# gaoyubin/EasyDarwin

Measured on AMD Instinct MI355X. Metric: relayed RTP packets/sec (whole node) + achieved HBM GB/s, 1080p H.264 fan-out, higher is better.
Workload: dtype u8

## Files before the change

### easydarwin_amd/csrc/edgpu_device.h

```cpp
#pragma once
#include <stdint.h>

namespace edgpu {

enum : uint32_t {
    kMaxPacket = 2060,
    kSlotWordsMax = 129,
    kIngestThreads = 256,
    kMaxTracks = 16,
    kMaxSendersPerSession = 2 * kMaxTracks,
};

enum : uint32_t {
    kSndRtcpPort = 1u << 0,
    kSndRtcpKind = 1u << 1,
    kSndVideo    = 1u << 2,
    kSndH264     = 1u << 3,
    kSndAudio    = 1u << 4,
};

struct PktMeta {
    uint64_t vbyte;
    uint64_t id;
    int64_t  arrival;
// ... 233 lines not shown

struct TickTotals {
    unsigned long long relayed_packets;
    unsigned long long relayed_bytes;
    unsigned long long arena_bytes;
    unsigned long long ing_pk[2], ing_b[2];
    int status;
    unsigned int nwork;
    unsigned long long cum_relayed_packets;
    unsigned long long cum_relayed_bytes;
    unsigned long long cum_fanout_in_bytes;
    unsigned long long cum_ingested_packets;
    unsigned long long cum_ingested_bytes;
    int ingest_status;
    unsigned int fan_next;
    unsigned int _pad;
    unsigned long long pass_bytes[2];
    unsigned int pass_desc[2];
    unsigned int pass_next[2];
    unsigned int pass_slot;
    unsigned int stream_errors;
    unsigned long long cum_lost_passes;
    unsigned int grow_count;
    unsigned int _pad_g;
};

struct GrowReq {
    uint32_t sender;
    uint32_t pk_log2;
    uint32_t bytes_log2;
    uint32_t _pad;
    uint64_t tail, head;
};
constexpr uint32_t kMaxGrow = 1024;
constexpr uint32_t kNoPass = 0xFFFFFFFFu;

struct TickParams {
    int64_t  now;
    int64_t  over_buffer_ms;
    uint64_t arena_bytes;
    uint32_t max_desc;
    uint32_t nsenders;
    uint32_t nsubs;
    uint32_t nsub_blocks;
    uint32_t chunk;
    uint32_t pass_ord;
    uint32_t pass_id;
    uint32_t grow_on;
    uint32_t grow_max_pk;
    uint64_t grow_max_bytes;
    uint32_t* grow_flag;
};

}
```

### easydarwin_amd/csrc/edgpu_engine.cpp

```cpp
#include <hip/hip_runtime.h>

#include <algorithm>
#include <cctype>
#include <chrono>
#include <thread>
#include <cstdio>
#include <cstdlib>
#include <cstring>
#include <map>
#include <mutex>
#include <string>
#include <vector>

#include <sched.h>

#include "edgpu.h"
#include "edgpu_device.h"

#include "edgpu_params.h"

namespace edgpu {
hipError_t launch_ingest(const IngestParams& p, uint32_t nseg, hipStream_t st);
hipError_t launch_blocked(const BlockedParams& p, hipStream_t st);
hipError_t launch_first_packet_info(const FirstInfoQuery* q, FirstInfoResult* r, const SenderDev* senders,
// ... 250 lines not shown
    uint64_t work_cap_needed = 0;
    void* d_null = nullptr;

    DevVec<SessionDev> d_sessions;
    DevVec<SenderDev> d_senders;
    DevVec<StreamDev> d_streams;
    DevVec<StatDev> d_stats;
    uint32_t n_stats = 0;
    struct TapHost { void* rec = nullptr; void* unit = nullptr; uint64_t cap = 0; uint32_t sender = 0; };
    DevVec<TapDev> d_taps;
    std::map<uint32_t, TapHost> taps;
    std::vector<std::pair<uint32_t, uint64_t>> tap_grown;
    bool tap_list_dirty = false;
    DevVec<uint32_t> d_tap_list, d_tap_items;
    DevVec<uint8_t> d_tap_out;
    DevVec<edgpu_tap_unit> d_tap_units;
    DevVec<edgpu_tap_stream> d_tap_streams;
    TapPlace* d_tap_place = nullptr;
    DevVec<uint8_t> d_ts_es, d_ts_out;
    DevVec<edgpu_tap_unit> d_ts_units_in;
    DevVec<TsRange> d_ts_ranges;
    DevVec<edgpu_ts_state> d_ts_states;
    DevVec<TsRec> d_ts_recs;
    DevVec<uint32_t> d_ts_base;
    DevVec<edgpu_ts_unit> d_ts_rows;
    uint8_t* d_ts_fixed = nullptr;
    DevVec<SubDev> d_subs;
    DevVec<uint32_t> d_sub_index;
    DevVec<uint32_t> d_sub_range;
    DevVec<uint32_t> d_sub_pos;
    DevVec<FanSub> d_fansub;
    DevVec<edgpu_substream_out> d_sub_out;
    DevVec<FanWork> d_work;
    DevVec<uint64_t> d_blk_bytes;
    DevVec<uint32_t> d_blk_count;
    DevVec<uint64_t> d_blk_maxb;
    DevVec<uint32_t> d_blk_maxc;
    bool index_dirty = true;
    uint32_t pass_ord = 0, pass_id = 0;
    int passes_more = 0;
    int tick_variant = 0;
    uint64_t fanout_passes = 0;

    edgpu_pkt_desc* d_desc = nullptr;
    uint32_t* d_seg = nullptr;
    uint32_t* d_seg_sess = nullptr;
    uint8_t* d_blob = nullptr;
    struct PinStage {
        edgpu_pkt_desc* desc = nullptr;
        uint32_t* seg = nullptr;
        uint32_t* sess = nullptr;
        uint8_t* blob = nullptr;
        hipEvent_t copied = nullptr;
        hipEvent_t consumed = nullptr;
        bool issued = false;
        uint64_t prestaged = 0;
    } pin[2];
    hipStream_t h2d = nullptr;
    int pin_next = 0;
    std::mutex pin_mu;
    int pend_stage = -1;
    const uint32_t* pend_seg = nullptr;
    const uint32_t* pend_seg_sess = nullptr;
    uint32_t pend_nseg = 0;
    bool pending = false;

    uint8_t* d_arena = nullptr;
    edgpu_out_desc* d_out_desc = nullptr;
    std::vector<uint32_t> carry_len;
    DevVec<uint8_t> d_carry;
// ... 189 lines not shown
    if (dmalloc(&x->d_seg, sizeof(uint32_t) * ((size_t)c.max_batch_packets + 1)) != hipSuccess) return bad("seg staging");
    if (dmalloc(&x->d_seg_sess, sizeof(uint32_t) * (size_t)c.max_batch_packets) != hipSuccess) return bad("seg staging");
    if (dmalloc(&x->d_arena, c.out_arena_bytes) != hipSuccess) return bad("fan-out arena");
    if (dmalloc(&x->d_out_desc, sizeof(edgpu_out_desc) * (size_t)c.max_out_packets) != hipSuccess) return bad("descriptors");
    if (dmalloc(&x->d_totals, sizeof(TickTotals)) != hipSuccess) return bad("totals");
    if (dmalloc(&x->d_grow, sizeof(GrowReq) * kMaxGrow) != hipSuccess) return bad("ring growth requests");
    if (hipHostMalloc((void**)&x->h_grow_flag, 64, hipHostMallocMapped) != hipSuccess ||
        hipHostGetDevicePointer((void**)&x->d_grow_flag, x->h_grow_flag, 0) != hipSuccess)
        return bad("ring growth flag");
    *x->h_grow_flag = 0;
    if (hipMalloc(&x->d_null, 4096) != hipSuccess || hipMemset(x->d_null, 0, 4096) != hipSuccess) return bad("null ring");
    {
        TickTotals t0;
        memset(&t0, 0, sizeof(t0));
        t0.pass_next[0] = t0.pass_next[1] = kNoPass;
        if (hipMemcpy(x->d_totals, &t0, sizeof(t0), hipMemcpyHostToDevice) != hipSuccess) return bad("totals");
    }
    if (const char* v = getenv("EDGPU_FANOUT")) x->fanout_variant = atoi(v);
    if (const char* v = getenv("EDGPU_TCP_WALK"))
        x->tcp_walk = !strcmp(v, "serial") || !strcmp(v, "1") ? 1u : !strcmp(v, "seg") || !strcmp(v, "2") ? 2u : 0u;
    if (const char* v = getenv("EDGPU_TCP_SEG")) x->tcp_seg = (uint32_t)std::max(atoi(v), 1);
    *out = x;
    return EDGPU_OK;
}

int edgpu_ctx_destroy(edgpu_ctx* x) {
    if (!x) return EDGPU_OK;
    (void)hipSetDevice(x->device);
    if (x->stream) (void)hipStreamSynchronize(x->stream);
    x->rings.release();
    if (x->d_null) (void)hipFree(x->d_null);
    x->d_sessions.release(); x->d_senders.release(); x->d_streams.release(); x->d_stats.release(); x->d_subs.release();
    x->d_sub_index.release(); x->d_sub_range.release(); x->d_sub_pos.release(); x->d_fansub.release(); x->d_sub_out.release(); x->d_work.release();
    x->d_blk_bytes.release(); x->d_blk_count.release(); x->d_blk_maxb.release(); x->d_blk_maxc.release();
    x->d_img_plan.release();
    for (auto& t : x->taps) { (void)hipFree(t.second.rec); (void)hipFree(t.second.unit); }
    x->d_taps.release(); x->d_tap_list.release(); x->d_tap_items.release(); x->d_tap_out.release();
    x->d_tap_units.release(); x->d_tap_streams.release();
    if (x->d_tap_place) (void)hipFree(x->d_tap_place);
    x->d_ts_es.release(); x->d_ts_out.release(); x->d_ts_units_in.release(); x->d_ts_ranges.release();
    x->d_ts_states.release(); x->d_ts_recs.release(); x->d_ts_base.release(); x->d_ts_rows.release();
    if (x->d_ts_fixed) (void)hipFree(x->d_ts_fixed);
    x->d_carry.release(); x->d_tcp_groups.release(); x->d_tcp_reads.release(); x->d_tcp_chunk_group.release();
    x->d_tcp_ncand.release(); x->d_tcp_cands.release(); x->d_tcp_links.release(); x->d_tcp_chunkres.release();
    x->d_tcp_results.release(); x->d_tcp_offs.release(); x->d_tcp_stage.release(); x->d_blocked.release();
    x->d_gather_reg.release(); x->d_gather_off.release(); x->d_arrivals.release(); x->d_sources.release(); x->d_row_sel.release(); x->d_rows.release();
    x->d_act_blk.release(); x->d_act_q.release(); x->d_act_rows.release();
    if (x->d_fpi_q) (void)hipFree(x->d_fpi_q);
    if (x->d_fpi_r) (void)hipFree(x->d_fpi_r);
    if (x->h_fpi_q) (void)hipHostFree(x->h_fpi_q);
    if (x->h_fpi_r) (void)hipHostFree(x->h_fpi_r);
    if (x->h_stage) (void)hipHostFree(x->h_stage);
    if (x->h_grow_flag) (void)hipHostFree(x->h_grow_flag);
    if (x->d_tcp_src) (void)hipFree(x->d_tcp_src);
    if (x->d_tcp_tot) (void)hipFree(x->d_tcp_tot);
    if (x->d_tcp_raw) (void)hipFree(x->d_tcp_raw);
    if (x->d_img_status) (void)hipFree(x->d_img_status);
    for (void* p : {(void*)x->d_desc, (void*)x->d_seg, (void*)x->d_seg_sess,
                    (void*)x->d_blob, (void*)x->d_arena, (void*)x->d_out_desc, (void*)x->d_totals, (void*)x->d_grow})
        if (p) (void)hipFree(p);
    for (auto& w : x->hist) for (auto& s : w) for (auto& e : s) if (e) (void)hipEventDestroy(e);
    if (x->h2d) (void)hipStreamSynchronize(x->h2d);
    for (auto& st : x->pin) {
        for (void* p : {(void*)st.desc, (void*)st.seg, (void*)st.sess, (void*)st.blob}) if (p) (void)hipFree(p);
        if (st.copied) (void)hipEventDestroy(st.copied);
        if (st.consumed) (void)hipEventDestroy(st.consumed);
    }
// ... 836 lines not shown
    }
    return true;
}

static int rebuild_index(edgpu_ctx* x) {
    const uint32_t nsub = (uint32_t)x->sub_sender.size();
    std::vector<uint32_t> range(2 * (size_t)x->nsenders, 0);
    for (uint32_t i = 0; i < nsub; i++)
        if (x->sub_active[i]) range[2 * (size_t)x->sub_sender[i] + 1]++;
    uint32_t total = 0;
    for (uint32_t s = 0; s < x->nsenders; s++) {
        const uint32_t c = range[2 * (size_t)s + 1];
        range[2 * (size_t)s] = total;
        range[2 * (size_t)s + 1] = total;
        total += c;
    }
    std::vector<uint32_t> idx(total);
    std::vector<uint32_t> pos(nsub, 0xFFFFFFFFu);
    for (uint32_t i = 0; i < nsub; i++)
        if (x->sub_active[i]) {
            const uint32_t k = range[2 * (size_t)x->sub_sender[i] + 1]++;
            idx[k] = i;
            pos[i] = k;
        }
    HIP_CHECK(x->d_sub_index.reserve(std::max<size_t>(idx.size(), 1), x->stream));
    HIP_CHECK(x->d_fansub.reserve(std::max<size_t>(idx.size(), 1), x->stream));
    HIP_CHECK(x->d_sub_pos.reserve(std::max<size_t>(nsub, 1), x->stream));
    if (nsub) HIP_CHECK(hipMemcpyAsync(x->d_sub_pos.ptr, pos.data(), nsub * 4, hipMemcpyHostToDevice, x->stream));
    HIP_CHECK(x->d_sub_range.reserve(std::max<size_t>(range.size(), 2), x->stream));
    if (!idx.empty()) HIP_CHECK(hipMemcpyAsync(x->d_sub_index.ptr, idx.data(), idx.size() * 4, hipMemcpyHostToDevice, x->stream));
    if (!range.empty()) HIP_CHECK(hipMemcpyAsync(x->d_sub_range.ptr, range.data(), range.size() * 4, hipMemcpyHostToDevice, x->stream));
    const uint32_t nblk = (nsub + 255) / 256;
    HIP_CHECK(x->d_sub_out.reserve(std::max<uint32_t>(nsub, 1), x->stream));
    HIP_CHECK(x->d_blk_bytes.reserve(std::max<uint32_t>(nblk, 1), x->stream));
    HIP_CHECK(x->d_blk_count.reserve(std::max<uint32_t>(nblk, 1), x->stream));
    HIP_CHECK(x->d_blk_maxb.reserve(std::max<uint32_t>(nblk, 1), x->stream));
    HIP_CHECK(x->d_blk_maxc.reserve(std::max<uint32_t>(nblk, 1), x->stream));
    HIP_CHECK(x->d_work.reserve(std::max<uint64_t>(x->work_cap_needed, 1), x->stream));
    HIP_CHECK(wsync(x, x->stream));
    x->index_dirty = false;
    return EDGPU_OK;
}

static int enqueue_ingest(edgpu_ctx* x, const edgpu_pkt_desc* dd, uint32_t n, const uint32_t* ds, const uint32_t* dss,
                          uint32_t nseg, const uint8_t* db, bool host_src, const TcpParams* tcp = nullptr,
                          bool deframed = false) {
    IngestParams p;
    p.host_epoch = host_src ? ++x->ingest_epoch : 0u;
    if (!host_src) ++x->ingest_epoch;
    x->host_epoch_last = p.host_epoch;
    p.desc = dd; p.seg_off = ds; p.seg_sess = dss; p.blob = db;
    p.src_addr = tcp ? tcp->src_addr : nullptr;
    p.sessions = x->d_sessions.ptr; p.senders = x->d_senders.ptr; p.streams = x->d_streams.ptr;
    p.npk = n; p.spec_min = x->cfg.ingest_spec_min;
    p.totals = x->d_totals;
    x->ing_slot ^= 1u;
    p.ing_slot = x->ing_slot;
    p.recv_time = x->cfg.reflector_use_in_packet_receive_time;
    p.max_future_ms = (int64_t)(uint32_t)(x->cfg.reflector_in_packet_max_receive_sec * 1000u);
    p.tcp_groups = tcp ? tcp->groups : nullptr;
    p.tcp_chunkres = tcp ? tcp->chunkres : nullptr;
    p.tcp_offs = tcp ? tcp->offs : nullptr;
    p.tcp_reads = tcp ? tcp->reads : nullptr;
    p.tcp_raw = tcp ? tcp->raw : nullptr;
    p.tcp_stage = tcp ? tcp->stage : nullptr;
    HIP_CHECK(hist_mark(x, 2, 0));
    if (tcp && !deframed) HIP_CHECK(launch_deframe(*tcp, x->stream));
    HIP_CHECK(launch_ingest(p, nseg, x->stream));
    HIP_CHECK(hist_mark(x, 2, 1));
    if (x->n_stats) {
// ... 294 lines not shown
}

int edgpu_keyframe_index(edgpu_ctx* x) {
    if (!x) return fail(EDGPU_BAD_ARGUMENT, "ctx is NULL");
    if (!x->pending) return fail(EDGPU_ERR, "no ingested batch pending a keyframe index");
    DEVICE_ENTER(x);
    x->kf_share = false;
    if (x->aux) {
        HIP_CHECK(hipEventRecord(x->ev_kf, x->stream));
        x->kf_recorded = true;
    }
    if (x->pend_stage >= 0) {
        HIP_CHECK(hipEventRecord(x->pin[x->pend_stage].consumed, x->stream));
        x->pend_stage = -1;
    }
    x->pending = false;
    return EDGPU_OK;
}

static int pick_fanout_variant(const edgpu_ctx* x) {
    if (x->fanout_variant >= 0) return x->fanout_variant;
    constexpr uint64_t kBurstRows = 4096;
    const bool burst = x->joined_rows >= kBurstRows && x->joined_rows * 4 >= x->sub_sender.size();
    return fanout_default(x->n_rw + x->n_tcp > 0 || burst);
}

static PlanParams plan_params(edgpu_ctx* x, int64_t now_ms) {
    const uint32_t nsub = x->tick_nsubs;
    PlanParams p;
    p.senders = x->d_senders.ptr; p.subs = x->d_subs.ptr; p.sub_index = x->d_sub_index.ptr;
    p.sub_pos = x->d_sub_pos.ptr; p.sub_range = x->d_sub_range.ptr; p.fansub = x->d_fansub.ptr;
    p.sub_out = x->d_sub_out.ptr;
    p.work = x->d_work.ptr;
    p.blk_bytes = x->d_blk_bytes.ptr; p.blk_count = x->d_blk_count.ptr;
    p.blk_maxb = x->d_blk_maxb.ptr; p.blk_maxc = x->d_blk_maxc.ptr;
    p.sessions = x->d_sessions.ptr;
    p.totals = x->d_totals;
    p.T.now = now_ms;
    p.T.over_buffer_ms = (int64_t)x->cfg.reflector_buffer_size_sec * 1000;
    p.T.arena_bytes = x->cfg.out_arena_bytes;
    p.T.max_desc = x->cfg.max_out_packets;
    p.T.nsenders = x->nsenders;
    p.T.nsubs = nsub;
    p.T.nsub_blocks = (nsub + 255) / 256;
    p.T.chunk = (uint32_t)fanout_chunk(x->tick_variant);
    p.T.pass_ord = x->pass_ord;
    p.T.pass_id = x->pass_id;
    p.grow = x->d_grow;
    p.T.grow_on = x->cfg.ring_growth;
    p.T.grow_max_pk = x->cfg.max_ring_packets;
    p.T.grow_max_bytes = x->cfg.max_ring_bytes;
    p.T.grow_flag = x->d_grow_flag;
    return p;
}

static int launch_copy_pass(edgpu_ctx* x, edgpu_fanout_result* out) {
    FanoutParams f;
    f.senders = x->d_senders.ptr; f.sub_range = x->d_sub_range.ptr; f.subs = x->d_subs.ptr;
    f.sub_index = x->d_sub_index.ptr; f.work = x->d_work.ptr; f.fansub = x->d_fansub.ptr;
    f.arena = x->d_arena; f.desc = x->d_out_desc;
    f.arena_words = x->cfg.out_arena_bytes / 16;
    f.max_desc = x->cfg.max_out_packets;
    f.totals = x->d_totals;
    hipStream_t cs = x->stream;
    HIP_CHECK(hist_mark(x, 0, 0, cs));
    HIP_CHECK(launch_fanout(f, x->tick_variant, x->num_cus, cs));
    HIP_CHECK(hist_mark(x, 0, 1, cs));
    x->fanout_passes++;
    x->passes_more = -1;
    if (out) {
        out->arena = f.arena;
        out->desc = f.desc;
        out->substreams = x->d_sub_out.ptr;
        out->n_substreams = x->tick_nsubs;
    }
    return EDGPU_OK;
}

int edgpu_fanout(edgpu_ctx* x, int64_t now_ms, edgpu_fanout_result* out) {
    if (!x) return fail(EDGPU_BAD_ARGUMENT, "ctx is NULL");
    if (x->pending) return fail(EDGPU_ERR, "edgpu_keyframe_index must run after edgpu_ingest");
    if (int r = owed_pass(x, "edgpu_fanout")) return r;
    DEVICE_ENTER(x);
    for (const auto& f : x->free_pending) x->free_subs[f.first].push_back(f.second);
    x->free_pending.clear();
    if (x->index_dirty) { int r = rebuild_index(x); if (r) return r; }
    x->tick_nsubs = (uint32_t)x->sub_sender.size();
    x->last_now = now_ms;
    queue_source_reports(x, now_ms);
    x->tick_variant = pick_fanout_variant(x);
    x->joined_rows = 0;
    x->pass_ord = 0;
    x->pass_id = 0;
    const PlanParams p = plan_params(x, now_ms);
    HIP_CHECK(hist_mark(x, 1, 0));
    HIP_CHECK(launch_plan(p, x->stream));
    if (int r = launch_copy_pass(x, out)) return r;
    if (x->timing >= EDGPU_TIMING_ALL) {
        const uint32_t s1 = x->hist_n[1];
        x->tick_end[s1 % edgpu_ctx::kHist] = x->last_seq[0];
        x->last_seq[1] = s1;
        x->hist_n[1] = s1 + 1;
    }
    x->fanout_launches++;
    x->timed_fanout = true;
    return EDGPU_OK;
}

int edgpu_fanout_next(edgpu_ctx* x, edgpu_fanout_result* out, uint32_t* launched) {
    if (!x || !launched) return fail(EDGPU_BAD_ARGUMENT, "NULL argument");
    *launched = 0;
    if (x->fanout_launches == 0) return fail(EDGPU_ERR, "no fan-out tick");
    DEVICE_ENTER(x);
    TickTotals t;
    if (int r = read_totals(x, &t)) return r;
    note_grow(x, t);
    if (t.status) {
        x->passes_more = 0;
        return fail(t.status, "the tick failed");
    }
    const uint32_t next = t.pass_next[x->pass_ord & 1u];
    if (next == kNoPass) {
        x->passes_more = 0;
        return EDGPU_OK;
    }
    x->pass_ord++;
    x->pass_id = next;
    const PlanParams p = plan_params(x, x->last_now);
    HIP_CHECK(launch_plan_pass(p, x->stream));
// ... 954 lines not shown
```

### easydarwin_amd/csrc/edgpu_kernels.hip

```cpp
#include <hip/hip_runtime.h>
#include <stdint.h>
#include "edgpu.h"
#include "edgpu_device.h"
#include "edgpu_params.h"
#include "edgpu_bytes.h"

namespace edgpu {

typedef unsigned int u32x4 __attribute__((ext_vector_type(4)));

__device__ __forceinline__ u32x4 ing_ld(const u32x4* p) { return *p; }
__device__ __forceinline__ void ing_st(u32x4* p, u32x4 v) { *p = v; }

__device__ __forceinline__ uint32_t be16(const uint8_t* p) { return (uint32_t)p[0] << 8 | p[1]; }
__device__ __forceinline__ uint32_t be32(const uint8_t* p) {
    return (uint32_t)p[0] << 24 | (uint32_t)p[1] << 16 | (uint32_t)p[2] << 8 | p[3];
}

__device__ __forceinline__ uint32_t slot_header(uint32_t len) {
    return 0x24u | ((len >> 8) & 0xFF) << 16 | (len & 0xFF) << 24;
}

__device__ bool key_frame_first_packet(const uint8_t* p, uint32_t len) {
    if (len < 20) return false;
// ... 694 lines not shown
    return lo;
}
__device__ uint64_t wave_first_arrival_at(const SenderDev& D, const PktMeta* meta, uint64_t lo, uint64_t hi, int64_t cut) {
    if (!D.rt_nonmono)
        return wave_lower_bound_meta(meta, D.pk_mask, lo, hi, [&](const PktMeta& m) { return m.arrival >= cut; });
    const uint64_t lane = threadIdx.x & 63;
    for (uint64_t b = lo; b < hi; b += 64) {
        const uint64_t i = b + lane;
        const unsigned long long t = __ballot(i < hi && meta[i & D.pk_mask].arrival >= cut ? 1 : 0);
        if (t) return b + (uint64_t)(__ffsll(t) - 1);
    }
    return hi;
}

__device__ __forceinline__ void reset_tick_totals(TickTotals* t) {
    t->relayed_packets = 0; t->relayed_bytes = 0; t->arena_bytes = 0;
    t->status = 0; t->nwork = 0; t->fan_next = 0; t->stream_errors = 0;
    if (t->pass_next[t->pass_slot & 1u] != kNoPass) t->cum_lost_passes++;
    t->pass_slot = 0;
    for (int k = 0; k < 2; k++) { t->pass_bytes[k] = 0; t->pass_desc[k] = 0; t->pass_next[k] = kNoPass; }
    t->grow_count = 0;
}

__global__ void k_totals_reset(TickTotals* t, int which) {
    if (threadIdx.x != 0) return;
    if (which == 0) reset_tick_totals(t);
    else for (int k = 0; k < 2; k++) { t->ing_pk[k] = 0; t->ing_b[k] = 0; }
}

__device__ __forceinline__ void mark_stream_error(const PlanParams& P, uint32_t session) {
    if (atomicOr(&P.sessions[session].errors, kStreamRingOverflow) == 0u) atomicAdd(&P.totals->stream_errors, 1u);
}

__global__ __launch_bounds__(256) void k_plan_senders(PlanParams P) {
    if (blockIdx.x == 0 && threadIdx.x == 0) reset_tick_totals(P.totals);
    const uint32_t s = blockIdx.x * (blockDim.x / 64) + threadIdx.x / 64;
    if (s >= P.T.nsenders) return;
    SenderDev& D = P.senders[s];
    const PktMeta* meta = reinterpret_cast<const PktMeta*>(D.meta);
    const uint64_t head = D.head;
    const uint64_t pk_cap = (uint64_t)D.pk_mask + 1;
    const uint64_t byte_cap = ((uint64_t)D.word_mask + 1) * 16;
    uint64_t lo = head > pk_cap ? head - pk_cap : 0;
    lo = max(lo, D.floor);
    const uint64_t vend = D.vbyte_end, vhigh = max(vend, D.vclob);
    const uint64_t tail = wave_lower_bound_meta(meta, D.pk_mask, lo, head,
                                                [&](const PktMeta& m) { return vhigh - m.vbyte <= byte_cap; });
    int64_t ns = -1;
    if (D.key >= 0) {
        ns = D.key;
        if ((uint64_t)ns < tail) ns = -2;
    } else if (head > tail) {
        const int64_t cutoff = P.T.now - P.T.over_buffer_ms;
        const uint64_t f = wave_first_arrival_at(D, meta, tail, head, cutoff);
        if (f < head) ns = (f == tail && tail > D.floor) ? -2 : (int64_t)f;
    }
    if (P.T.grow_on && head > tail) {
        const uint64_t held_b = vend - meta[tail & D.pk_mask].vbyte;
        if (2 * (head - tail) > pk_cap || 2 * held_b > byte_cap) {
            const int64_t age_cut = P.T.now - 10 * P.T.over_buffer_ms;
            uint64_t r = wave_first_arrival_at(D, meta, tail, head, age_cut);
            if (D.key >= 0 && (uint64_t)D.key >= tail) r = min(r, (uint64_t)D.key);
            if (D.umin >= tail) r = min(r, D.umin);
            const uint64_t need_pk = head - r;
            const uint64_t need_b = r < head ? vend - meta[r & D.pk_mask].vbyte : 0;
            uint64_t want_pk = pk_cap, want_b = byte_cap;
            while (2 * need_pk > want_pk && want_pk < P.T.grow_max_pk) want_pk *= 2;
            while (2 * need_b > want_b && want_b < P.T.grow_max_bytes) want_b *= 2;
            if ((threadIdx.x & 63) == 0 && (want_pk > pk_cap || want_b > byte_cap)) {
                const uint32_t k = atomicAdd(&P.totals->grow_count, 1u);
                if (k < kMaxGrow)
                    P.grow[k] = GrowReq{s, (uint32_t)(63 - __clzll((long long)want_pk)),
                                        (uint32_t)(63 - __clzll((long long)want_b)), 0u, tail, head};
                if (k == 0 && P.T.grow_flag) *(volatile uint32_t*)P.T.grow_flag = 1u;
            }
        }
    }
    if ((threadIdx.x & 63) == 0) {
        D.tail = tail;
        D.new_start = ns;
        D.umin = head;
    }
}

template <typename T>
__global__ __launch_bounds__(256) void k_ring_move(const T* __restrict__ src, uint64_t smask, T* __restrict__ dst,
                                                   uint64_t dmask, uint64_t lo, uint64_t n) {
    for (uint64_t i = (uint64_t)blockIdx.x * 256 + threadIdx.x; i < n; i += (uint64_t)gridDim.x * 256) {
        const uint64_t v = lo + i;
        dst[v & dmask] = src[v & smask];
    }
}

__global__ __launch_bounds__(256) void k_plan_subs(PlanParams P) {
    const uint32_t q = blockIdx.x * blockDim.x + threadIdx.x;
    uint64_t bytes = 0;
    uint32_t count = 0;
    if (q < P.T.nsubs) {
        SubDev& Q = P.subs[q];
        Q.nonempty = 0; Q.count = 0; Q.bytes = 0;
        Q.was_new = Q.active && Q.bookmark < 0;
        if (Q.active) {
            SenderDev& D = P.senders[Q.sender];
            const PktMeta* meta = reinterpret_cast<const PktMeta*>(D.meta);
            const uint64_t head = D.head;
            bool have = false;
            uint64_t a = 0;
            Q.prev_last_id = Q.last_id;
            Q.prev_has_last = Q.has_last;
            Q.prev_sent_any = Q.sent_any;
            if (Q.bookmark >= 0) {
                a = (uint64_t)Q.bookmark + (Q.resume_at ? 0u : 1u);
                if (Q.rtp_info && Q.kind == 0 && !Q.has_last && (Q.sent_any || P.subs[q + 1].sent_any))
                    a = (uint64_t)Q.bookmark;
                have = true;
                if (a < D.tail && a < head) { mark_stream_error(P, D.session); a = D.tail; }
            } else if (D.new_start >= 0) {
                a = (uint64_t)D.new_start;
                have = true;
                if (Q.has_last)
                    a = lower_bound_meta(meta, D.pk_mask, a, head,
                                         [&](const PktMeta& m) { return m.id > Q.last_id; });
            } else if (D.new_start == -2) {
                mark_stream_error(P, D.session);
            }
            if (have) {
                if (Q.rtp_info && Q.kind == 0 && !Q.sent_any && !P.subs[q + 1].sent_any) {
                    while (a < head) {
                        const PktMeta m = meta[a & D.pk_mask];
                        if (m.len != 0 && m.seq >= Q.first_seq) break;
                        a++;
                    }
                }
                if (a < head) {
                    const PktMeta m = meta[a & D.pk_mask];
                    Q.a = a;
                    Q.vstart = m.vbyte;
                    Q.vcstart = m.vcount;
                    bytes = D.vbyte_end - m.vbyte;
                    count = D.vcount_end - m.vcount;
                    Q.bytes = bytes;
                    Q.count = count;
                    Q.nonempty = 1;
                    atomicMin((unsigned long long*)&D.umin, (unsigned long long)a);
                }
                if (head > 0) { Q.bookmark = (int64_t)(head - 1); Q.resume_at = 0; }
                if (count > 0) {
                    Q.last_id = meta[(uint64_t)D.last_nonzero & D.pk_mask].id;
                    Q.has_last = 1;
                }
            }
        }
    }
    __shared__ uint64_t sb[4];
    __shared__ uint32_t sc[4];
    uint64_t tb; uint32_t tc;
    (void)block_exclusive_scan<uint64_t>(bytes, sb, tb);
    (void)block_exclusive_scan<uint32_t>(count, sc, tc);
    const uint64_t mb = block_reduce<uint64_t, OpMax>(bytes, sb);
    const uint32_t mc = block_reduce<uint32_t, OpMax>(count, sc);
    if (threadIdx.x == 0) {
        P.blk_bytes[blockIdx.x] = tb; P.blk_count[blockIdx.x] = tc;
        P.blk_maxb[blockIdx.x] = mb; P.blk_maxc[blockIdx.x] = mc;
    }
}

template <typename T>
__device__ __forceinline__ T wave_block_inclusive_scan(T v, T* wsum) {
    const int lane = threadIdx.x & 63, w = threadIdx.x >> 6;
#pragma unroll
    for (int o = 1; o < 64; o <<= 1) {
        const T y = __shfl_up(v, o, 64);
        if (lane >= o) v += y;
    }
    if (lane == 63) wsum[w] = v;
    __syncthreads();
    T base = 0;
    for (int i = 0; i < w; i++) base += wsum[i];
    __syncthreads();
    return v + base;
}

__global__ __launch_bounds__(256) void k_plan_final(PlanParams P) {
    const uint32_t q = blockIdx.x * blockDim.x + threadIdx.x;
    __shared__ uint64_t sb[4];
    __shared__ uint32_t sc[4];
    const uint32_t lane = threadIdx.x & 63;
    const uint32_t nwaves = gridDim.x * (blockDim.x / 64);
    const uint32_t gw = blockIdx.x * (blockDim.x / 64) + threadIdx.x / 64;
    auto chunks_of = [&](const SenderDev& D) {
        return (uint32_t)(((D.head > D.umin ? D.head - D.umin : 0) + P.T.chunk - 1) / P.T.chunk);
    };
    uint64_t bytes = 0; uint32_t count = 0;
    if (q < P.T.nsubs) { bytes = P.subs[q].bytes; count = P.subs[q].count; }
    uint32_t res_nch = 0, res_base = 0;
    if (gw + lane * nwaves < P.T.nsenders) res_nch = chunks_of(P.senders[gw + lane * nwaves]);
    uint64_t base_b, tb_all, mb;
    uint32_t base_c, tc_all, mc;
    {
        const uint32_t nb = P.T.nsub_blocks;
        uint64_t xb = 0, xba = 0, xmb = 0;
        uint32_t xc = 0, xca = 0, xmc = 0;
        for (uint32_t i = threadIdx.x; i < nb; i += blockDim.x) {
            const uint64_t b = P.blk_bytes[i];
            const uint32_t c = P.blk_count[i];
            xba += b; xca += c;
            if (i < blockIdx.x) { xb += b; xc += c; }
            xmb = max(xmb, P.blk_maxb[i]); xmc = max(xmc, P.blk_maxc[i]);
        }
        base_b = block_reduce<uint64_t, OpSum>(xb, sb); tb_all = block_reduce<uint64_t, OpSum>(xba, sb);
        mb = block_reduce<uint64_t, OpMax>(xmb, sb);
        base_c = block_reduce<uint32_t, OpSum>(xc, sc); tc_all = block_reduce<uint32_t, OpSum>(xca, sc);
        mc = block_reduce<uint32_t, OpMax>(xmc, sc);
    }
    const bool fits = tb_all <= P.T.arena_bytes && tc_all <= P.T.max_desc;
    const bool impossible = mb > P.T.arena_bytes || mc > P.T.max_desc;
    const uint64_t W = (fits || impossible) ? 16ull : ((P.T.arena_bytes - mb) & ~15ull) + 16;
    const uint32_t Wc = (fits || impossible) ? 1u : P.T.max_desc - mc + 1;
    if (blockIdx.x == 0 && threadIdx.x == 0) {
        P.totals->arena_bytes = tb_all;
        P.totals->relayed_packets = tc_all;
        P.totals->cum_relayed_packets += tc_all;
        if (!fits && impossible) atomicExch(&P.totals->status, EDGPU_OUT_OVERFLOW);
        if (fits) { P.totals->pass_bytes[0] = tb_all; P.totals->pass_desc[0] = tc_all; }
    }
    uint64_t tb; uint32_t tc;
    const uint64_t pb = block_exclusive_scan<uint64_t>(bytes, sb, tb);
    const uint32_t pc = block_exclusive_scan<uint32_t>(count, sc, tc);
    uint64_t end_b = 0; uint32_t end_c = 0, next = kNoPass;
    if (q < P.T.nsubs) {
        SubDev& Q = P.subs[q];
        uint64_t ob = base_b + pb;
        uint32_t od = base_c + pc, pass = 0;
        if (!fits) {
            const uint64_t kb = ob / W;
            const uint32_t kc = od / Wc;
            pass = (uint32_t)kb + kc;
            ob -= kb * W;
            od -= kc * Wc;
        }
        Q.out_base = ob;
        Q.desc_base = od;
// ... 876 lines not shown


hipError_t launch_ingest(const IngestParams& p, uint32_t nseg, hipStream_t st) {
    if (nseg == 0) {
        EDGPU_LAUNCH(k_totals_reset, dim3(1), dim3(64), 0, st, p.totals, 1);
        return hipGetLastError();
    }
    const bool spec = !p.tcp_groups && !p.src_addr && p.spec_min && p.npk >= (uint64_t)p.spec_min * nseg;
    if (spec) EDGPU_LAUNCH(k_ingest<true>, dim3(nseg), dim3(kIngestThreads), 0, st, p);
    else EDGPU_LAUNCH(k_ingest<false>, dim3(nseg), dim3(kIngestThreads), 0, st, p);
    return hipGetLastError();
}
hipError_t launch_image(const ImageParams& p, int phase, hipStream_t st) {
    if (p.nplan == 0) return hipSuccess;
    if (phase == 0) EDGPU_LAUNCH(k_image_plan, dim3((p.nplan + 255) / 256), dim3(256), 0, st, p);
    else if (phase == 1) EDGPU_LAUNCH(k_image_pack, dim3(p.nplan), dim3(256), 0, st, p);
    else if (phase == 2) EDGPU_LAUNCH(k_image_apply, dim3(p.nplan), dim3(256), 0, st, p);
    else EDGPU_LAUNCH(k_image_fit, dim3((p.nplan + 255) / 256), dim3(256), 0, st, p);
    return hipGetLastError();
}
hipError_t launch_first_packet_info(const FirstInfoQuery* q, FirstInfoResult* r, const SenderDev* senders,
                                    uint32_t n, hipStream_t st) {
    if (n == 0) return hipSuccess;
    EDGPU_LAUNCH(k_first_packet_info, dim3((n + 63) / 64), dim3(64), 0, st, q, r, senders, n);
    return hipGetLastError();
}
hipError_t launch_blocked(const BlockedParams& p, hipStream_t st) {
    if (p.n) EDGPU_LAUNCH(k_blocked, dim3((p.n + 63) / 64), dim3(64), 0, st, p);
    return hipGetLastError();
}

hipError_t launch_plan(const PlanParams& p, hipStream_t st) {
    const uint32_t nsb = p.T.nsenders ? (p.T.nsenders + 255) / 256 : 0;
    if (nsb) EDGPU_LAUNCH(k_plan_senders, dim3((p.T.nsenders + 3) / 4), dim3(256), 0, st, p);
    else EDGPU_LAUNCH(k_totals_reset, dim3(1), dim3(64), 0, st, p.totals, 0);
    if (p.T.nsub_blocks) EDGPU_LAUNCH(k_plan_subs, dim3(p.T.nsub_blocks), dim3(256), 0, st, p);
    const uint32_t nfb = max(p.T.nsub_blocks, nsb);
    if (nfb) EDGPU_LAUNCH(k_plan_final, dim3(nfb), dim3(256), 0, st, p);
    return hipGetLastError();
}
hipError_t launch_ring_move(int kind, const void* src, uint64_t smask, void* dst, uint64_t dmask, uint64_t lo, uint64_t n,
                            hipStream_t st) {
    if (!n) return hipSuccess;
    const uint64_t nb = (n + 255) / 256;
    const uint32_t blocks = (uint32_t)(nb < 4096 ? nb : 4096);
    if (kind == 0)
        EDGPU_LAUNCH(k_ring_move<PktMeta>, dim3(blocks), dim3(256), 0, st, (const PktMeta*)src, smask, (PktMeta*)dst, dmask, lo, n);
    else if (kind == 1)
        EDGPU_LAUNCH(k_ring_move<uint32_t>, dim3(blocks), dim3(256), 0, st, (const uint32_t*)src, smask, (uint32_t*)dst, dmask, lo, n);
    else
        EDGPU_LAUNCH(k_ring_move<u32x4>, dim3(blocks), dim3(256), 0, st, (const u32x4*)src, smask, (u32x4*)dst, dmask, lo, n);
    return hipGetLastError();
}
hipError_t launch_plan_pass(const PlanParams& p, hipStream_t st) {
    EDGPU_LAUNCH(k_plan_pass, dim3(max(p.T.nsub_blocks, 1u)), dim3(256), 0, st, p);
    return hipGetLastError();
}
static int occupancy_of(const void* fn, int threads, int lds) {
    int blocks = 0;
    if (hipOccupancyMaxActiveBlocksPerMultiprocessor(&blocks, fn, threads, lds) != hipSuccess) return 1;
    return blocks > 0 ? blocks : 1;
}
struct FanoutVariant { const void* fn; int threads; int chunk; int lds; };
static const FanoutVariant kVariants[] = {
    {(const void*)k_fanout4<1024, 32>, 1024, 32, fanout4_lds<1024, 32>()},
    {(const void*)k_fanout6<1024, 16>, 1024, 16, fanout6_lds<1024, 16>()},
};
static const char* const kVariantNames[] = {"k_fanout4<1024,32,nt,dyn>", "k_fanout6<1024,16,nt,dyn>"};
static const int kNumVariants = sizeof(kVariants) / sizeof(kVariants[0]);
// ... 27 lines not shown
```

### easydarwin_amd/csrc/edgpu_params.h

```cpp
#pragma once
#include <stdint.h>
#include "edgpu.h"
#include "edgpu_device.h"

namespace edgpu {

extern thread_local uint64_t tl_launches;
#define EDGPU_LAUNCH(...)                          \
    do {                                           \
        ++::edgpu::tl_launches;                    \
        hipLaunchKernelGGL(__VA_ARGS__);           \
    } while (0)

constexpr uint32_t kTcpFramesPerRound = 4;

struct TcpGroup;
struct TcpChunkRes;
struct TcpRead;

struct IngestParams {
    const edgpu_pkt_desc* desc;
    const uint32_t* seg_off;
    const uint32_t* seg_sess;
    const uint8_t* blob;
    const uint64_t* src_addr;
    SessionDev* sessions;
    SenderDev* senders;
    StreamDev* streams;
    uint32_t npk;
    uint32_t spec_min;
    uint32_t host_epoch;
    TickTotals* totals;
    uint32_t ing_slot;
    uint32_t recv_time;
    int64_t max_future_ms;
    const TcpGroup* tcp_groups;
    const TcpChunkRes* tcp_chunkres;
    const uint16_t* tcp_offs;
    const TcpRead* tcp_reads;
    const uint8_t* tcp_raw;
    const uint8_t* tcp_stage;
};

struct PlanParams {
    SenderDev* senders;
    SubDev* subs;
    const uint32_t* sub_index;
    const uint32_t* sub_pos;
    const uint32_t* sub_range;
    edgpu_substream_out* sub_out;
    FanWork* work;
    FanSub* fansub;
    uint64_t* blk_bytes;
    uint32_t* blk_count;
    uint64_t* blk_maxb;
    uint32_t* blk_maxc;
    SessionDev* sessions;
    TickTotals* totals;
    GrowReq* grow;
    TickParams T;
};

struct FanoutParams {
    const SenderDev* senders;
    const uint32_t* sub_range;
    const SubDev* subs;
    const uint32_t* sub_index;
    const FanWork* work;
    const FanSub* fansub;
    uint8_t* arena;
    edgpu_out_desc* desc;
    uint64_t arena_words;
    uint32_t max_desc;
    TickTotals* totals;
};

#ifndef EDGPU_TCP_CHUNK
#define EDGPU_TCP_CHUNK 32768
#endif
constexpr uint32_t kTcpChunk = EDGPU_TCP_CHUNK;
#ifndef EDGPU_TCP_SPEC
#define EDGPU_TCP_SPEC 0
#endif
constexpr uint32_t kTcpSpec = EDGPU_TCP_SPEC;
#ifndef EDGPU_TCP_CAND_FUSED
#define EDGPU_TCP_CAND_FUSED 0
#endif
#ifndef EDGPU_TCP_WALK_CPW
#define EDGPU_TCP_WALK_CPW 2
// ... 146 lines not shown
```

Measured before the change: 3.361 billion.

## Fuse sender and subscriber planning into one kernel with double-buffered atomic partials

Merges k_plan_senders and k_plan_subs into a single k_plan_tick kernel in which each sender's wavefront plans its own subscribers, so one launch and one round trip of sender state through memory go away. Per-block byte/count sums and maxima are now built with wave-level reductions and atomics into double-buffered PlanPart slots. The final kernel reads these slots and clears the other parity for the next tick, and a host-side parity bit flips each tick. The cost is that subscriber work is now serialized per sender wavefront, which load-balances poorly when a sender has many subscribers, and it adds atomics plus a dependence on the parity toggle staying consistent.

```diff
diff --git a/easydarwin_amd/csrc/edgpu_device.h b/easydarwin_amd/csrc/edgpu_device.h
--- a/easydarwin_amd/csrc/edgpu_device.h
+++ b/easydarwin_amd/csrc/edgpu_device.h
@@ -289,6 +289,12 @@
     uint32_t _pad;
     uint64_t tail, head;
 };
+struct PlanPart {
+    unsigned long long bytes;
+    unsigned long long maxb;
+    uint32_t count;
+    uint32_t maxc;
+};
 constexpr uint32_t kMaxGrow = 1024;
 constexpr uint32_t kNoPass = 0xFFFFFFFFu;
 
@@ -303,6 +309,7 @@
     uint32_t chunk;
     uint32_t pass_ord;
     uint32_t pass_id;
+    uint32_t plan_par;
     uint32_t grow_on;
     uint32_t grow_max_pk;
     uint64_t grow_max_bytes;
diff --git a/easydarwin_amd/csrc/edgpu_engine.cpp b/easydarwin_amd/csrc/edgpu_engine.cpp
--- a/easydarwin_amd/csrc/edgpu_engine.cpp
+++ b/easydarwin_amd/csrc/edgpu_engine.cpp
@@ -306,10 +306,9 @@
     DevVec<FanSub> d_fansub;
     DevVec<edgpu_substream_out> d_sub_out;
     DevVec<FanWork> d_work;
-    DevVec<uint64_t> d_blk_bytes;
-    DevVec<uint32_t> d_blk_count;
-    DevVec<uint64_t> d_blk_maxb;
-    DevVec<uint32_t> d_blk_maxc;
+    DevVec<PlanPart> d_plan_part;
+    uint32_t plan_part_blocks = 0;
+    uint32_t plan_par = 0;
     bool index_dirty = true;
     uint32_t pass_ord = 0, pass_id = 0;
     int passes_more = 0;
@@ -565,7 +564,7 @@
     if (x->d_null) (void)hipFree(x->d_null);
     x->d_sessions.release(); x->d_senders.release(); x->d_streams.release(); x->d_stats.release(); x->d_subs.release();
     x->d_sub_index.release(); x->d_sub_range.release(); x->d_sub_pos.release(); x->d_fansub.release(); x->d_sub_out.release(); x->d_work.release();
-    x->d_blk_bytes.release(); x->d_blk_count.release(); x->d_blk_maxb.release(); x->d_blk_maxc.release();
+    x->d_plan_part.release();
     x->d_img_plan.release();
     for (auto& t : x->taps) { (void)hipFree(t.second.rec); (void)hipFree(t.second.unit); }
     x->d_taps.release(); x->d_tap_list.release(); x->d_tap_items.release(); x->d_tap_out.release();
@@ -1468,10 +1467,11 @@
     if (!range.empty()) HIP_CHECK(hipMemcpyAsync(x->d_sub_range.ptr, range.data(), range.size() * 4, hipMemcpyHostToDevice, x->stream));
     const uint32_t nblk = (nsub + 255) / 256;
     HIP_CHECK(x->d_sub_out.reserve(std::max<uint32_t>(nsub, 1), x->stream));
-    HIP_CHECK(x->d_blk_bytes.reserve(std::max<uint32_t>(nblk, 1), x->stream));
-    HIP_CHECK(x->d_blk_count.reserve(std::max<uint32_t>(nblk, 1), x->stream));
-    HIP_CHECK(x->d_blk_maxb.reserve(std::max<uint32_t>(nblk, 1), x->stream));
-    HIP_CHECK(x->d_blk_maxc.reserve(std::max<uint32_t>(nblk, 1), x->stream));
+    HIP_CHECK(x->d_plan_part.reserve(2 * (size_t)std::max<uint32_t>(nblk, 1), x->stream));
+    if (nblk != x->plan_part_blocks || !x->plan_part_blocks) {
+        HIP_CHECK(hipMemsetAsync(x->d_plan_part.ptr, 0, x->d_plan_part.cap * sizeof(PlanPart), x->stream));
+        x->plan_part_blocks = nblk;
+    }
     HIP_CHECK(x->d_work.reserve(std::max<uint64_t>(x->work_cap_needed, 1), x->stream));
     HIP_CHECK(wsync(x, x->stream));
     x->index_dirty = false;
@@ -1832,8 +1832,8 @@
     p.sub_pos = x->d_sub_pos.ptr; p.sub_range = x->d_sub_range.ptr; p.fansub = x->d_fansub.ptr;
     p.sub_out = x->d_sub_out.ptr;
     p.work = x->d_work.ptr;
-    p.blk_bytes = x->d_blk_bytes.ptr; p.blk_count = x->d_blk_count.ptr;
-    p.blk_maxb = x->d_blk_maxb.ptr; p.blk_maxc = x->d_blk_maxc.ptr;
+    p.part = x->d_plan_part.ptr;
+    p.T.plan_par = x->plan_par;
     p.sessions = x->d_sessions.ptr;
     p.totals = x->d_totals;
     p.T.now = now_ms;
@@ -1895,6 +1895,7 @@
     const PlanParams p = plan_params(x, now_ms);
     HIP_CHECK(hist_mark(x, 1, 0));
     HIP_CHECK(launch_plan(p, x->stream));
+    if (p.T.nsenders || p.T.nsub_blocks) x->plan_par ^= 1u;
     if (int r = launch_copy_pass(x, out)) return r;
     if (x->timing >= EDGPU_TIMING_ALL) {
         const uint32_t s1 = x->hist_n[1];
diff --git a/easydarwin_amd/csrc/edgpu_kernels.hip b/easydarwin_amd/csrc/edgpu_kernels.hip
--- a/easydarwin_amd/csrc/edgpu_kernels.hip
+++ b/easydarwin_amd/csrc/edgpu_kernels.hip
@@ -750,10 +750,84 @@
     if (atomicOr(&P.sessions[session].errors, kStreamRingOverflow) == 0u) atomicAdd(&P.totals->stream_errors, 1u);
 }
 
-__global__ __launch_bounds__(256) void k_plan_senders(PlanParams P) {
+template <typename T>
+__global__ __launch_bounds__(256) void k_ring_move(const T* __restrict__ src, uint64_t smask, T* __restrict__ dst,
+                                                   uint64_t dmask, uint64_t lo, uint64_t n) {
+    for (uint64_t i = (uint64_t)blockIdx.x * 256 + threadIdx.x; i < n; i += (uint64_t)gridDim.x * 256) {
+        const uint64_t v = lo + i;
+        dst[v & dmask] = src[v & smask];
+    }
+}
+
+__device__ __forceinline__ void plan_sub_row(const PlanParams& P, uint32_t q, const SenderDev& D, const PktMeta* meta,
+                                             uint64_t head, uint64_t tail, int64_t ns, uint64_t& bytes, uint32_t& count,
+                                             uint64_t& amin) {
+    SubDev& Q = P.subs[q];
+    Q.nonempty = 0; Q.count = 0; Q.bytes = 0;
+    Q.was_new = Q.active && Q.bookmark < 0;
+    if (!Q.active) return;
+    bool have = false;
+    uint64_t a = 0;
+    Q.prev_last_id = Q.last_id;
+    Q.prev_has_last = Q.has_last;
+    Q.prev_sent_any = Q.sent_any;
+    if (Q.bookmark >= 0) {
+        a = (uint64_t)Q.bookmark + (Q.resume_at ? 0u : 1u);
+        if (Q.rtp_info && Q.kind == 0 && !Q.has_last && (Q.sent_any || P.subs[q + 1].sent_any))
+            a = (uint64_t)Q.bookmark;
+        have = true;
+        if (a < tail && a < head) { mark_stream_error(P, D.session); a = tail; }
+    } else if (ns >= 0) {
+        a = (uint64_t)ns;
+        have = true;
+        if (Q.has_last)
+            a = lower_bound_meta(meta, D.pk_mask, a, head,
+                                 [&](const PktMeta& m) { return m.id > Q.last_id; });
+    } else if (ns == -2) {
+        mark_stream_error(P, D.session);
+    }
+    if (!have) return;
+    if (Q.rtp_info && Q.kind == 0 && !Q.sent_any && !P.subs[q + 1].sent_any) {
+        while (a < head) {
+            const PktMeta m = meta[a & D.pk_mask];
+            if (m.len != 0 && m.seq >= Q.first_seq) break;
+            a++;
+        }
+    }
+    if (a < head) {
+        const PktMeta m = meta[a & D.pk_mask];
+        Q.a = a;
+        Q.vstart = m.vbyte;
+        Q.vcstart = m.vcount;
+        bytes = D.vbyte_end - m.vbyte;
+        count = D.vcount_end - m.vcount;
+        Q.bytes = bytes;
+        Q.count = count;
+        Q.nonempty = 1;
+        amin = min(amin, a);
+    }
+    if (head > 0) { Q.bookmark = (int64_t)(head - 1); Q.resume_at = 0; }
+    if (count > 0) {
+        Q.last_id = meta[(uint64_t)D.last_nonzero & D.pk_mask].id;
+        Q.has_last = 1;
+    }
+}
+
+__global__ __launch_bounds__(256) void k_plan_tick(PlanParams P) {
     if (blockIdx.x == 0 && threadIdx.x == 0) reset_tick_totals(P.totals);
+    const uint32_t nsb = (P.T.nsenders + 3) / 4;
+    if (blockIdx.x >= nsb) {
+        const uint32_t q = (blockIdx.x - nsb) * blockDim.x + threadIdx.x;
+        if (q < P.T.nsubs && P.sub_pos[q] == 0xFFFFFFFFu) {
+            SubDev& Q = P.subs[q];
+            Q.nonempty = 0; Q.count = 0; Q.bytes = 0;
+            Q.was_new = Q.active && Q.bookmark < 0;
+        }
+        return;
+    }
     const uint32_t s = blockIdx.x * (blockDim.x / 64) + threadIdx.x / 64;
     if (s >= P.T.nsenders) return;
+    const uint32_t lane = threadIdx.x & 63;
     SenderDev& D = P.senders[s];
     const PktMeta* meta = reinterpret_cast<const PktMeta*>(D.meta);
     const uint64_t head = D.head;
@@ -785,7 +859,7 @@
             uint64_t want_pk = pk_cap, want_b = byte_cap;
             while (2 * need_pk > want_pk && want_pk < P.T.grow_max_pk) want_pk *= 2;
             while (2 * need_b > want_b && want_b < P.T.grow_max_bytes) want_b *= 2;
-            if ((threadIdx.x & 63) == 0 && (want_pk > pk_cap || want_b > byte_cap)) {
+            if (lane == 0 && (want_pk > pk_cap || want_b > byte_cap)) {
                 const uint32_t k = atomicAdd(&P.totals->grow_count, 1u);
                 if (k < kMaxGrow)
                     P.grow[k] = GrowReq{s, (uint32_t)(63 - __clzll((long long)want_pk)),
@@ -794,92 +868,47 @@
             }
         }
     }
-    if ((threadIdx.x & 63) == 0) {
+    const uint32_t qb = P.sub_range[2 * s], qe = P.sub_range[2 * s + 1];
+    uint64_t amin = head;
+    for (uint32_t base = qb; base < qe; base += 64) {
+        const uint32_t pos = base + lane;
+        uint32_t q = 0, count = 0;
+        uint64_t bytes = 0;
+        if (pos < qe) {
+            q = P.sub_index[pos];
+            plan_sub_row(P, q, D, meta, head, tail, ns, bytes, count, amin);
+        }
+        const uint32_t blk = (bytes | count) ? q >> 8 : 0xFFFFFFFFu;
+        unsigned long long todo = __ballot(blk != 0xFFFFFFFFu ? 1 : 0);
+        while (todo) {
+            const int leader = __ffsll(todo) - 1;
+            const uint32_t b = (uint32_t)__shfl((int)blk, leader, 64);
+            const bool mine = blk == b;
+            uint64_t tb = mine ? bytes : 0, mb = tb;
+            uint32_t tc = mine ? count : 0, mc = tc;
+#pragma unroll
+            for (int o = 32; o > 0; o >>= 1) {
+                tb += (uint64_t)__shfl_xor(tb, o, 64);
+                tc += (uint32_t)__shfl_xor(tc, o, 64);
+                mb = max(mb, (uint64_t)__shfl_xor(mb, o, 64));
+                mc = max(mc, (uint32_t)__shfl_xor(mc, o, 64));
+            }
+            if ((int)lane == leader) {
+                PlanPart& R = P.part[2 * b + P.T.plan_par];
+                atomicAdd(&R.bytes, (unsigned long long)tb);
+                atomicAdd(&R.count, tc);
+                atomicMax(&R.maxb, (unsigned long long)mb);
+                atomicMax(&R.maxc, mc);
+            }
+            todo &= ~__ballot(mine ? 1 : 0);
+        }
+    }
+#pragma unroll
+    for (int o = 32; o > 0; o >>= 1) amin = min(amin, (uint64_t)__shfl_xor(amin, o, 64));
+    if (lane == 0) {
         D.tail = tail;
         D.new_start = ns;
-        D.umin = head;
-    }
-}
-
-template <typename T>
-__global__ __launch_bounds__(256) void k_ring_move(const T* __restrict__ src, uint64_t smask, T* __restrict__ dst,
-                                                   uint64_t dmask, uint64_t lo, uint64_t n) {
-    for (uint64_t i = (uint64_t)blockIdx.x * 256 + threadIdx.x; i < n; i += (uint64_t)gridDim.x * 256) {
-        const uint64_t v = lo + i;
-        dst[v & dmask] = src[v & smask];
-    }
-}
-
-__global__ __launch_bounds__(256) void k_plan_subs(PlanParams P) {
-    const uint32_t q = blockIdx.x * blockDim.x + threadIdx.x;
-    uint64_t bytes = 0;
-    uint32_t count = 0;
-    if (q < P.T.nsubs) {
-        SubDev& Q = P.subs[q];
-        Q.nonempty = 0; Q.count = 0; Q.bytes = 0;
-        Q.was_new = Q.active && Q.bookmark < 0;
-        if (Q.active) {
-            SenderDev& D = P.senders[Q.sender];
-            const PktMeta* meta = reinterpret_cast<const PktMeta*>(D.meta);
-            const uint64_t head = D.head;
-            bool have = false;
-            uint64_t a = 0;
-            Q.prev_last_id = Q.last_id;
-            Q.prev_has_last = Q.has_last;
-            Q.prev_sent_any = Q.sent_any;
-            if (Q.bookmark >= 0) {
-                a = (uint64_t)Q.bookmark + (Q.resume_at ? 0u : 1u);
-                if (Q.rtp_info && Q.kind == 0 && !Q.has_last && (Q.sent_any || P.subs[q + 1].sent_any))
-                    a = (uint64_t)Q.bookmark;
-                have = true;
-                if (a < D.tail && a < head) { mark_stream_error(P, D.session); a = D.tail; }
-            } else if (D.new_start >= 0) {
-                a = (uint64_t)D.new_start;
-                have = true;
-                if (Q.has_last)
-                    a = lower_bound_meta(meta, D.pk_mask, a, head,
-                                         [&](const PktMeta& m) { return m.id > Q.last_id; });
-            } else if (D.new_start == -2) {
-                mark_stream_error(P, D.session);
-            }
-            if (have) {
-                if (Q.rtp_info && Q.kind == 0 && !Q.sent_any && !P.subs[q + 1].sent_any) {
-                    while (a < head) {
-                        const PktMeta m = meta[a & D.pk_mask];
-                        if (m.len != 0 && m.seq >= Q.first_seq) break;
-                        a++;
-                    }
-                }
-                if (a < head) {
-                    const PktMeta m = meta[a & D.pk_mask];
-                    Q.a = a;
-                    Q.vstart = m.vbyte;
-                    Q.vcstart = m.vcount;
-                    bytes = D.vbyte_end - m.vbyte;
-                    count = D.vcount_end - m.vcount;
-                    Q.bytes = bytes;
-                    Q.count = count;
-                    Q.nonempty = 1;
-                    atomicMin((unsigned long long*)&D.umin, (unsigned long long)a);
-                }
-                if (head > 0) { Q.bookmark = (int64_t)(head - 1); Q.resume_at = 0; }
-                if (count > 0) {
-                    Q.last_id = meta[(uint64_t)D.last_nonzero & D.pk_mask].id;
-                    Q.has_last = 1;
-                }
-            }
-        }
-    }
-    __shared__ uint64_t sb[4];
-    __shared__ uint32_t sc[4];
-    uint64_t tb; uint32_t tc;
-    (void)block_exclusive_scan<uint64_t>(bytes, sb, tb);
-    (void)block_exclusive_scan<uint32_t>(count, sc, tc);
-    const uint64_t mb = block_reduce<uint64_t, OpMax>(bytes, sb);
-    const uint32_t mc = block_reduce<uint32_t, OpMax>(count, sc);
-    if (threadIdx.x == 0) {
-        P.blk_bytes[blockIdx.x] = tb; P.blk_count[blockIdx.x] = tc;
-        P.blk_maxb[blockIdx.x] = mb; P.blk_maxc[blockIdx.x] = mc;
+        D.umin = amin;
     }
 }
 
@@ -920,12 +949,14 @@
         uint64_t xb = 0, xba = 0, xmb = 0;
         uint32_t xc = 0, xca = 0, xmc = 0;
         for (uint32_t i = threadIdx.x; i < nb; i += blockDim.x) {
-            const uint64_t b = P.blk_bytes[i];
-            const uint32_t c = P.blk_count[i];
+            const PlanPart R = P.part[2 * i + P.T.plan_par];
+            const uint64_t b = R.bytes;
+            const uint32_t c = R.count;
             xba += b; xca += c;
             if (i < blockIdx.x) { xb += b; xc += c; }
-            xmb = max(xmb, P.blk_maxb[i]); xmc = max(xmc, P.blk_maxc[i]);
-        }
+            xmb = max(xmb, (uint64_t)R.maxb); xmc = max(xmc, R.maxc);
+        }
+        if (threadIdx.x == 0 && blockIdx.x < nb) P.part[2 * blockIdx.x + (P.T.plan_par ^ 1u)] = PlanPart{0, 0, 0, 0};
         base_b = block_reduce<uint64_t, OpSum>(xb, sb); tb_all = block_reduce<uint64_t, OpSum>(xba, sb);
         mb = block_reduce<uint64_t, OpMax>(xmb, sb);
         base_c = block_reduce<uint32_t, OpSum>(xc, sc); tc_all = block_reduce<uint32_t, OpSum>(xca, sc);
@@ -1868,9 +1899,9 @@
 
 hipError_t launch_plan(const PlanParams& p, hipStream_t st) {
     const uint32_t nsb = p.T.nsenders ? (p.T.nsenders + 255) / 256 : 0;
-    if (nsb) EDGPU_LAUNCH(k_plan_senders, dim3((p.T.nsenders + 3) / 4), dim3(256), 0, st, p);
+    const uint32_t ntb = (p.T.nsenders + 3) / 4 + p.T.nsub_blocks;
+    if (ntb) EDGPU_LAUNCH(k_plan_tick, dim3(ntb), dim3(256), 0, st, p);
     else EDGPU_LAUNCH(k_totals_reset, dim3(1), dim3(64), 0, st, p.totals, 0);
-    if (p.T.nsub_blocks) EDGPU_LAUNCH(k_plan_subs, dim3(p.T.nsub_blocks), dim3(256), 0, st, p);
     const uint32_t nfb = max(p.T.nsub_blocks, nsb);
     if (nfb) EDGPU_LAUNCH(k_plan_final, dim3(nfb), dim3(256), 0, st, p);
     return hipGetLastError();
diff --git a/easydarwin_amd/csrc/edgpu_params.h b/easydarwin_amd/csrc/edgpu_params.h
--- a/easydarwin_amd/csrc/edgpu_params.h
+++ b/easydarwin_amd/csrc/edgpu_params.h
@@ -51,10 +51,7 @@
     edgpu_substream_out* sub_out;
     FanWork* work;
     FanSub* fansub;
-    uint64_t* blk_bytes;
-    uint32_t* blk_count;
-    uint64_t* blk_maxb;
-    uint32_t* blk_maxc;
+    PlanPart* part;
     SessionDev* sessions;
     TickTotals* totals;
     GrowReq* grow;
```

Result: no change. 3.398 billion, median of 3 (+1.1%).
